# waldstein94/Stratified-Transformer

Measured on AMD Instinct MI355X. Metric: points/sec through StratifiedAttention fwd+bwd, 100k-pt scene, higher is better.
Workload: dtype f32

## Files before the change

stratified_transformer_amd/csrc/cell_attn.hip:

```cpp
#include "cell_common.h"

namespace p2 {


template <typename T>
__device__ __forceinline__ void stage_table_t(T *lds, const T *__restrict__ tab, int L, int h, int head) {
    const int total = 3 * L * 16;
    for (int x = threadIdx.x; x < total; x += blockDim.x) {
        const int i = x % 16, r = (x / 16) % L, ax = x / (16 * L);
        lds[x] = tab[(((size_t)r * h + head) * 16 + i) * 3 + ax];
    }
}
template <int TS, typename T>
__device__ __forceinline__ void stage_tables(T *lds, const T *__restrict__ table_q, const T *__restrict__ table_k, const T *__restrict__ table_v, int L,
                                             int h, int head) {
    stage_table_t<T>(lds, table_q, L, h, head);
    stage_table_t<T>(lds + TS, table_k, L, h, head);
    stage_table_t<T>(lds + 2 * TS, table_v, L, h, head);
    __syncthreads();
}

template <int LCAP>
struct TabGeo {
    static constexpr int TS = 3 * LCAP * 16;
    static constexpr size_t bytes(size_t elem) { return (size_t)3 * TS * elem; }
};
struct RowOff {
    int o0, o1, o2;
};
__device__ __forceinline__ RowOff row_off(unsigned w, int L, int c) {
    RowOff r;
    r.o0 = (int)(w & 255u) * 16 + 4 * c;
    r.o1 = (int)(L + ((w >> 8) & 255u)) * 16 + 4 * c;
    r.o2 = (int)(2 * L + ((w >> 16) & 255u)) * 16 + 4 * c;
    return r;
}
template <int OFF>
__device__ __forceinline__ float4 tsum_at(const float *lds, RowOff r) {
    return add4(add4(*reinterpret_cast<const float4 *>(lds + OFF + r.o0), *reinterpret_cast<const float4 *>(lds + OFF + r.o1)),
                *reinterpret_cast<const float4 *>(lds + OFF + r.o2));
}

struct Rows3 {
    float4 a, b, c;
};
template <int OFF, typename T>
__device__ __forceinline__ Rows3 rows_at(const T *lds, RowOff r) {
    Rows3 x;
    x.a = ld_row4(lds + OFF + r.o0);
    x.b = ld_row4(lds + OFF + r.o1);
    x.c = ld_row4(lds + OFF + r.o2);
    return x;
}
typedef float f32x2c __attribute__((ext_vector_type(2)));
__device__ __forceinline__ float4 padd4(float4 a, float4 b) {
    const f32x2c lo = f32x2c{a.x, a.y} + f32x2c{b.x, b.y}, hi = f32x2c{a.z, a.w} + f32x2c{b.z, b.w};
    return make_float4(lo.x, lo.y, hi.x, hi.y);
}
__device__ __forceinline__ float4 pfma4(float s, float4 a, float4 acc) {
    const f32x2c ss = f32x2c{s, s};
    const f32x2c lo = __builtin_elementwise_fma(ss, f32x2c{a.x, a.y}, f32x2c{acc.x, acc.y});
    const f32x2c hi = __builtin_elementwise_fma(ss, f32x2c{a.z, a.w}, f32x2c{acc.z, acc.w});
    return make_float4(lo.x, lo.y, hi.x, hi.y);
}
__device__ __forceinline__ float4 rsum(Rows3 r) { return padd4(padd4(r.a, r.b), r.c); }
__device__ __forceinline__ f32x2c pdot_acc(float4 a, float4 b, f32x2c acc) {
    acc = __builtin_elementwise_fma(f32x2c{a.x, a.y}, f32x2c{b.x, b.y}, acc);
    return __builtin_elementwise_fma(f32x2c{a.z, a.w}, f32x2c{b.z, b.w}, acc);
}
__device__ __forceinline__ float pdot4(float4 a, float4 b) {
    const f32x2c r = pdot_acc(a, b, f32x2c{0.f, 0.f});
    return r.x + r.y;
}

template <int NPMAX, typename F>
__device__ __forceinline__ void dispatch_passes(int np, F f) {
    if (np <= 2) f(std::integral_constant<int, 2>{});
    else if (np == 3) f(std::integral_constant<int, 3>{});
    else if (np == 4 || NPMAX <= 4) f(std::integral_constant<int, 4>{});
    else if constexpr (NPMAX > 4) {
        if (np <= 6) f(std::integral_constant<int, 6>{});
        else f(std::integral_constant<int, 8>{});
    }
}

template <typename TT, bool PK>
struct LaneCtx {
    const TT *lds;
    int L, lane, p, c, head, h, C, hoff, rs_packed;
    float qscale;
    __device__ __forceinline__ int rs() const { return PK ? rs_packed : C; }
    template <typename RT>
    __device__ __forceinline__ float4 q_row4(const RT *q, int i) const {
        if constexpr (PK) return scaled_row4<RT>(q + (size_t)i * rs_packed + hoff, qscale);
        else return ld_row4(q + (size_t)i * C + hoff);
    }
};
template <typename TT, bool PK>
__device__ __forceinline__ LaneCtx<TT, PK> make_lane_ctx(const TT *lds, int h, int L, int rs, float qscale) {
    LaneCtx<TT, PK> x;
    x.lds = lds;
    x.L = L;
    x.h = h;
    x.head = blockIdx.y;
    x.C = h * 16;
    x.rs_packed = rs;
    x.qscale = qscale;
    x.lane = threadIdx.x & 63;
    x.p = x.lane >> 2;
    x.c = x.lane & 3;
    x.hoff = x.head * 16 + 4 * x.c;
    return x;
}

template <int NPA, typename RT, typename T, bool PK>
__device__ __forceinline__ void load_key_rows(const LaneCtx<T, PK> &x, const CellBufs &cb, const RT *__restrict__ rows, int j0, int nvalid,
                                              float4 (&r4)[NPA]) {
    unsigned keys[NPA];
    bload_words<NPA>(cb.key, (j0 + x.p * NPA) * 4, keys);
#pragma unroll
    for (int t = 0; t < NPA; t++) {
        const float4 r = ld_row4(rows + (size_t)keys[t] * x.rs() + x.hoff);
        r4[t] = t < nvalid ? r : make_float4(0.f, 0.f, 0.f, 0.f);
    }
}

template <int NPA, int TS, typename RT, typename T, bool PK>
__device__ __forceinline__ void fwd_sweep_logits(const LaneCtx<T, PK> &x, const CellTask &ct, const CellBufs &cb, rsrc_t rs_p,
                                                 const RT *__restrict__ q, const RT *__restrict__ k, float *__restrict__ ml,
                                                 int ch, bool single, int j0, int nkc) {
    const int p = x.p, c = x.c;
    const int nvalid = min(max(nkc - p * NPA, 0), NPA);
    float4 k4[NPA];
    load_key_rows<NPA, RT, T, PK>(x, cb, k, j0, nvalid, k4);
    int ids = (int)bload_u32(cb.qid, x.lane * 4);
    int i_nx = __builtin_amdgcn_readlane(ids, 0);
    float4 q4_nx = x.q_row4(q, i_nx);
    unsigned w_nx[NPA];
    bload_words<NPA>(cb.rel, (j0 + p * NPA) * 4, w_nx);
    for (int il = 0; il < ct.nq; il++) {
        const int i = i_nx;
        const float4 q4 = q4_nx;
        unsigned w[NPA];
#pragma unroll
        for (int t = 0; t < NPA; t++) w[t] = w_nx[t];
        const int roff = (il * ct.nk + j0 + p * NPA) * 4;
        if (((il + 1) & 63) == 0) ids = (int)bload_u32(cb.qid, (il + 1 + x.lane) * 4);
        i_nx = __builtin_amdgcn_readlane(ids, (il + 1) & 63);
        q4_nx = x.q_row4(q, i_nx);
        bload_words<NPA>(cb.rel, roff + ct.nk * 4, w_nx);
        float lg[NPA];
        float mx = -INFINITY;
        RowOff ro = row_off(w[0], x.L, c);
        Rows3 rq = rows_at<0, T>(x.lds, ro), rk = rows_at<TS, T>(x.lds, ro);
#pragma unroll
        for (int t = 0; t < NPA; t++) {
            Rows3 rq1 = rq, rk1 = rk;
            if (t + 1 < NPA) {
                ro = row_off(w[t + 1], x.L, c);
                rq1 = rows_at<0, T>(x.lds, ro);
                rk1 = rows_at<TS, T>(x.lds, ro);
            }
            const f32x2c d2 = pdot_acc(k4[t], rsum(rk), pdot_acc(q4, rsum(rq), pdot_acc(q4, k4[t], f32x2c{0.f, 0.f})));
            const float s = quad_sum(d2.x + d2.y);
            lg[t] = (t < nvalid && !(w[t] >> 31)) ? s : -INFINITY;
            mx = fmaxf(mx, lg[t]);
            rq = rq1;
            rk = rk1;
            __builtin_amdgcn_sched_barrier(0);
        }
        mx = slots_max16(mx);
        if (single) {
            float sum = 0.f;
#pragma unroll
            for (int t = 0; t < NPA; t++) {
                lg[t] = __expf(lg[t] - mx);
                sum += lg[t];
            }
            const float inv = 1.0f / slots_sum16(sum);
#pragma unroll
            for (int t = 0; t < NPA; t++) lg[t] *= inv;
            if (c == 0) bstore_floats<NPA>(rs_p, roff, lg, nvalid);
        } else {
            float *st = ml + ((size_t)i * x.h + x.head) * 2;
            const float m_old = ch ? st[0] : -INFINITY, l_old = ch ? st[1] : 0.f;
            const float m_new = fmaxf(m_old, mx);
            float sum = 0.f;
#pragma unroll
            for (int t = 0; t < NPA; t++) sum += __expf(lg[t] - m_new);
            if (c == 0) bstore_floats<NPA>(rs_p, roff, lg, nvalid);
            sum = slots_sum16(sum);
            if (x.lane == 0) {
                st[0] = m_new;
                st[1] = (m_old == -INFINITY ? 0.f : l_old * __expf(m_old - m_new)) + sum;
            }
        }
    }
}

template <int NPA, int TS, typename RT, typename T, bool PK>
__device__ __forceinline__ void fwd_sweep_values(const LaneCtx<T, PK> &x, const CellTask &ct, const CellBufs &cb, rsrc_t rs_p,
                                                 const RT *__restrict__ v, const float *__restrict__ ml, float *__restrict__ out,
                                                 int ch, bool single, int j0, int nkc) {
    const int p = x.p, c = x.c;
    const int nvalid = min(max(nkc - p * NPA, 0), NPA);
    float4 v4[NPA];
    load_key_rows<NPA, RT, T, PK>(x, cb, v, j0, nvalid, v4);
    unsigned w_nx[NPA];
    float a_nx[NPA];
    bload_words<NPA>(cb.rel, (j0 + p * NPA) * 4, w_nx);
    bload_floats<NPA>(rs_p, (j0 + p * NPA) * 4, a_nx);
    int ids = (int)bload_u32(cb.qid, x.lane * 4);
    for (int il = 0; il < ct.nq; il++) {
        if (il && (il & 63) == 0) ids = (int)bload_u32(cb.qid, (il + x.lane) * 4);
        const int i = __builtin_amdgcn_readlane(ids, il & 63);
        const int roff = (il * ct.nk + j0 + p * NPA) * 4;
        unsigned w[NPA];
        float a[NPA];
#pragma unroll
        for (int t = 0; t < NPA; t++) {
            w[t] = w_nx[t];
            a[t] = a_nx[t];
        }
        bload_words<NPA>(cb.rel, roff + ct.nk * 4, w_nx);
        bload_floats<NPA>(rs_p, roff + ct.nk * 4, a_nx);
        if (!single) {
            const float *st = ml + ((size_t)i * x.h + x.head) * 2;
            const float m = st[0], inv = 1.0f / st[1];
#pragma unroll
            for (int t = 0; t < NPA; t++) a[t] = __expf(a[t] - m) * inv;
            if (c == 0) bstore_floats<NPA>(rs_p, roff, a, nvalid);
        }
        float4 acc = make_float4(0.f, 0.f, 0.f, 0.f);
        Rows3 rv = rows_at<2 * TS, T>(x.lds, row_off(w[0], x.L, c));
#pragma unroll
        for (int t = 0; t < NPA; t++) {
            Rows3 rv1 = rv;
            if (t + 1 < NPA) rv1 = rows_at<2 * TS, T>(x.lds, row_off(w[t + 1], x.L, c));
            const float at = t < nvalid ? a[t] : 0.f;
            acc = pfma4(at, padd4(rsum(rv), v4[t]), acc);
            rv = rv1;
            __builtin_amdgcn_sched_barrier(0);
        }
        const float4 tot = slots_sum16_4(acc);
        if (p == 0) {
            float *o = out + (size_t)i * x.C + x.hoff;
            stg4(o, ch ? add4(tot, ldg4(o)) : tot);
        }
    }
}

template <int NP, int LCAP, typename RT, typename T, bool PK>
__global__ __launch_bounds__(CA_WAVES * 64) void cell_fwd_kernel(pointops2_cell_plan pl, int h, int L, const RT *__restrict__ q,
                                                                 const RT *__restrict__ k, const RT *__restrict__ v, int rs, float qscale,
                                                                 const T *__restrict__ table_q, const T *__restrict__ table_k,
                                                                 const T *__restrict__ table_v, float *__restrict__ out,
                                                                 float *__restrict__ ml, float *__restrict__ pbuf, size_t plane) {
    constexpr int TS = TabGeo<LCAP>::TS;
    extern __shared__ float lds_raw[];
    T *lds = reinterpret_cast<T *>(lds_raw);
    const LaneCtx<T, PK> x = make_lane_ctx<T, PK>(lds, h, L, rs, qscale);
    const int wave = __builtin_amdgcn_readfirstlane(threadIdx.x >> 6);
    stage_tables<TS, T>(lds, table_q, table_k, table_v, L, h, x.head);
    const int nC = share_count(pl, pl.counts[0]);
    float *pb = pbuf + (size_t)x.head * plane;
    const int slots = gridDim.x * CA_WAVES, slot = blockIdx.x * CA_WAVES + wave;
    for (int round = 0; round * slots < nC; round++) {
        const int task = snake_task(round, slot, slots);
        if (task >= nC) continue;
        const CellTask ct = cell_task(pl, share_task(pl, task));
        const int nch = (ct.nk + 16 * NP - 1) / (16 * NP);
        const CellBufs cb = make_cell_bufs(pl, ct);
        const rsrc_t rs_p = tile_rsrc(pb, ct);
        for (int ch = 0; ch < nch; ch++) {
            const int j0 = ch * 16 * NP, nkc = min(16 * NP, ct.nk - j0);
            dispatch_passes<NP>((nkc + 15) >> 4, [&](auto tag) {
                fwd_sweep_logits<decltype(tag)::value, TS, RT, T, PK>(x, ct, cb, rs_p, q, k, ml, ch, nch == 1, j0, nkc);
            });
        }
        for (int ch = 0; ch < nch; ch++) {
            const int j0 = ch * 16 * NP, nkc = min(16 * NP, ct.nk - j0);
            dispatch_passes<NP>((nkc + 15) >> 4, [&](auto tag) {
                fwd_sweep_values<decltype(tag)::value, TS, RT, T, PK>(x, ct, cb, rs_p, v, ml, out, ch, nch == 1, j0, nkc);
            });
        }
    }
}

template <int NPA, typename T, bool PK>
__device__ __forceinline__ void flush_key_pass(float *scr, float4 acc, rsrc_t rs_key, int j0, int t, int nkc, float *__restrict__ grad,
                                               const LaneCtx<T, PK> &x) {
    *reinterpret_cast<float4 *>(scr + x.p * 16 + 4 * x.c) = acc;
    __builtin_amdgcn_s_waitcnt(0xC07F);
    __builtin_amdgcn_wave_barrier();
#pragma unroll
    for (int kk = 0; kk < 4; kk++) {
        const int s = (x.lane >> 4) + 4 * kk;
        const int jl = s * NPA + t;
        const int key = (int)bload_u32(rs_key, (j0 + jl) * 4);
        if (jl < nkc) unsafeAtomicAdd(grad + (size_t)key * x.rs() + x.head * 16 + (x.lane & 15), scr[s * 16 + (x.lane & 15)]);
    }
    __builtin_amdgcn_s_waitcnt(0xC07F);
    __builtin_amdgcn_wave_barrier();
}

template <int NPA, int TS, typename RT, typename T, bool PK>
__device__ __forceinline__ void bwd_sweep_values(const LaneCtx<T, PK> &x, const CellTask &ct, const CellBufs &cb, rsrc_t rs_p, rsrc_t rs_g,
                                                 float *scr, const float *__restrict__ go, const float *__restrict__ out,
                                                 const RT *__restrict__ v, float *__restrict__ grad_v, int j0, int nkc) {
    const int p = x.p, c = x.c;
    const int nvalid = min(max(nkc - p * NPA, 0), NPA);
    float4 v4[NPA], dv4[NPA];
    load_key_rows<NPA, RT, T, PK>(x, cb, v, j0, nvalid, v4);
#pragma unroll
    for (int t = 0; t < NPA; t++) dv4[t] = make_float4(0.f, 0.f, 0.f, 0.f);
    unsigned w_nx[NPA];
    float a_nx[NPA];
    bload_words<NPA>(cb.rel, (j0 + p * NPA) * 4, w_nx);
    bload_floats<NPA>(rs_p, (j0 + p * NPA) * 4, a_nx);
    int ids = (int)bload_u32(cb.qid, x.lane * 4);
    int i_nx = __builtin_amdgcn_readlane(ids, 0);
    float4 go_nx = ldg4(go + (size_t)i_nx * x.C + x.hoff), o_nx = ldg4(out + (size_t)i_nx * x.C + x.hoff);
    for (int il = 0; il < ct.nq; il++) {
        const int roff = (il * ct.nk + j0 + p * NPA) * 4;
        const float4 go4 = go_nx, o4 = o_nx;
        unsigned w[NPA];
        float a[NPA];
#pragma unroll
        for (int t = 0; t < NPA; t++) {
            w[t] = w_nx[t];
            a[t] = t < nvalid ? a_nx[t] : 0.f;
        }
        if (((il + 1) & 63) == 0) ids = (int)bload_u32(cb.qid, (il + 1 + x.lane) * 4);
        i_nx = __builtin_amdgcn_readlane(ids, (il + 1) & 63);
        go_nx = ldg4(go + (size_t)i_nx * x.C + x.hoff);
        o_nx = ldg4(out + (size_t)i_nx * x.C + x.hoff);
        bload_words<NPA>(cb.rel, roff + ct.nk * 4, w_nx);
        bload_floats<NPA>(rs_p, roff + ct.nk * 4, a_nx);
        const float delta = quad_sum(pdot4(go4, o4));
        float gs[NPA];
        Rows3 rv = rows_at<2 * TS, T>(x.lds, row_off(w[0], x.L, c));
#pragma unroll
        for (int t = 0; t < NPA; t++) {
            Rows3 rv1 = rv;
            if (t + 1 < NPA) rv1 = rows_at<2 * TS, T>(x.lds, row_off(w[t + 1], x.L, c));
            const float ga = quad_sum(pdot4(go4, padd4(rsum(rv), v4[t])));
            gs[t] = a[t] * (ga - delta);
            dv4[t] = pfma4(a[t], go4, dv4[t]);
            rv = rv1;
            __builtin_amdgcn_sched_barrier(0);
        }
        if (c == 0) bstore_floats<NPA>(rs_g, roff, gs, nvalid);
    }
#pragma unroll
    for (int t = 0; t < NPA; t++) flush_key_pass<NPA, T, PK>(scr, dv4[t], cb.key, j0, t, nkc, grad_v, x);
}

template <int NPA, int TS, typename RT, typename T, bool PK>
__device__ __forceinline__ void bwd_sweep_keys(const LaneCtx<T, PK> &x, const CellTask &ct, const CellBufs &cb, rsrc_t rs_g, float *scr,
                                               const RT *__restrict__ q, const RT *__restrict__ k, float *__restrict__ grad_q,
                                               float *__restrict__ grad_k, int ch, int j0, int nkc) {
    const int p = x.p, c = x.c;
    const int nvalid = min(max(nkc - p * NPA, 0), NPA);
    float4 k4[NPA], dk4[NPA];
    load_key_rows<NPA, RT, T, PK>(x, cb, k, j0, nvalid, k4);
#pragma unroll
    for (int t = 0; t < NPA; t++) dk4[t] = make_float4(0.f, 0.f, 0.f, 0.f);
    unsigned w_nx[NPA];
    float g_nx[NPA];
    bload_words<NPA>(cb.rel, (j0 + p * NPA) * 4, w_nx);
    bload_floats<NPA>(rs_g, (j0 + p * NPA) * 4, g_nx);
    int ids = (int)bload_u32(cb.qid, x.lane * 4);
    int i_nx = __builtin_amdgcn_readlane(ids, 0);
    float4 q_nx = x.q_row4(q, i_nx);
    for (int il = 0; il < ct.nq; il++) {
        const int i = i_nx;
        const int roff = (il * ct.nk + j0 + p * NPA) * 4;
        const float4 q4 = q_nx;
        unsigned w[NPA];
        float g[NPA];
#pragma unroll
        for (int t = 0; t < NPA; t++) {
            w[t] = w_nx[t];
            g[t] = t < nvalid ? g_nx[t] : 0.f;
        }
        if (((il + 1) & 63) == 0) ids = (int)bload_u32(cb.qid, (il + 1 + x.lane) * 4);
        i_nx = __builtin_amdgcn_readlane(ids, (il + 1) & 63);
        q_nx = x.q_row4(q, i_nx);
        bload_words<NPA>(cb.rel, roff + ct.nk * 4, w_nx);
        bload_floats<NPA>(rs_g, roff + ct.nk * 4, g_nx);
        float4 dq = make_float4(0.f, 0.f, 0.f, 0.f);
        RowOff ro = row_off(w[0], x.L, c);
        Rows3 rq = rows_at<0, T>(x.lds, ro), rk = rows_at<TS, T>(x.lds, ro);
#pragma unroll
        for (int t = 0; t < NPA; t++) {
            Rows3 rq1 = rq, rk1 = rk;
            if (t + 1 < NPA) {
                ro = row_off(w[t + 1], x.L, c);
                rq1 = rows_at<0, T>(x.lds, ro);
                rk1 = rows_at<TS, T>(x.lds, ro);
            }
            dq = pfma4(g[t], padd4(rsum(rq), k4[t]), dq);
            dk4[t] = pfma4(g[t], padd4(rsum(rk), q4), dk4[t]);
            rq = rq1;
            rk = rk1;
            __builtin_amdgcn_sched_barrier(0);
        }
        float4 tot = slots_sum16_4(dq);
        if constexpr (PK) tot = make_float4(tot.x * x.qscale, tot.y * x.qscale, tot.z * x.qscale, tot.w * x.qscale);
        if (p == 0) {
            float *o = grad_q + (size_t)i * x.rs() + x.hoff;
            stg4(o, ch ? add4(tot, ldg4(o)) : tot);
        }
    }
#pragma unroll
    for (int t = 0; t < NPA; t++) flush_key_pass<NPA, T, PK>(scr, dk4[t], cb.key, j0, t, nkc, grad_k, x);
}

template <int NP, int LCAP, typename RT, typename T, bool PK>
__global__ __launch_bounds__(CA_WAVES_BWD * 64) void cell_bwd_kernel(pointops2_cell_plan pl, int h, int L, const float *__restrict__ go,
                                                                 const RT *__restrict__ q, const RT *__restrict__ k,
                                                                 const RT *__restrict__ v, int rs, float qscale, const float *__restrict__ out,
                                                                 const T *__restrict__ table_q, const T *__restrict__ table_k,
                                                                 const T *__restrict__ table_v, const float *__restrict__ pbuf,
                                                                 float *__restrict__ gsbuf, size_t plane, float *__restrict__ grad_q,
                                                                 float *__restrict__ grad_k, float *__restrict__ grad_v) {
    constexpr int TS = TabGeo<LCAP>::TS;
    extern __shared__ float lds_raw[];
    T *lds = reinterpret_cast<T *>(lds_raw);
    const LaneCtx<T, PK> x = make_lane_ctx<T, PK>(lds, h, L, rs, qscale);
    const int wave = __builtin_amdgcn_readfirstlane(threadIdx.x >> 6);
    float *scr = reinterpret_cast<float *>(lds + 3 * TS) + wave * 256;
    stage_tables<TS, T>(lds, table_q, table_k, table_v, L, h, x.head);
    const int nC = share_count(pl, pl.counts[0]);
    const float *pb = pbuf + (size_t)x.head * plane;
    float *gb = gsbuf + (size_t)x.head * plane;
    const int slots = gridDim.x * CA_WAVES_BWD, slot = blockIdx.x * CA_WAVES_BWD + wave;
    for (int round = 0; round * slots < nC; round++) {
        const int task = snake_task(round, slot, slots);
        if (task >= nC) continue;
        const CellTask ct = cell_task(pl, share_task(pl, task));
        const int nch = (ct.nk + 16 * NP - 1) / (16 * NP);
        const CellBufs cb = make_cell_bufs(pl, ct);
        const rsrc_t rs_p = tile_rsrc(pb, ct), rs_g = tile_rsrc(gb, ct);
        for (int ch = 0; ch < nch; ch++) {
            const int j0 = ch * 16 * NP, nkc = min(16 * NP, ct.nk - j0);
            dispatch_passes<NP>((nkc + 15) >> 4, [&](auto tag) {
                bwd_sweep_values<decltype(tag)::value, TS, RT, T, PK>(x, ct, cb, rs_p, rs_g, scr, go, out, v, grad_v, j0, nkc);
            });
        }
        for (int ch = 0; ch < nch; ch++) {
            const int j0 = ch * 16 * NP, nkc = min(16 * NP, ct.nk - j0);
            dispatch_passes<NP>((nkc + 15) >> 4, [&](auto tag) {
                bwd_sweep_keys<decltype(tag)::value, TS, RT, T, PK>(x, ct, cb, rs_g, scr, q, k, grad_q, grad_k, ch, j0, nkc);
            });
        }
    }
}

struct CFixScale {
    float mul, inv;
};
__device__ __forceinline__ CFixScale c_row_scale(unsigned maxbits, int n) {
    CFixScale sc;
    if (maxbits >= 0x7f800000u) {
        sc.mul = 0.f;
        sc.inv = __uint_as_float(0x7fc00000u);
        return sc;
    }
    const int E = (int)(maxbits >> 23) - 126;
    const int bits_n = 32 - __clz(max(n, 1));
    const int S = max(-126, min(126, 30 - bits_n - E));
    sc.mul = __uint_as_float((unsigned)(S + 127) << 23);
    sc.inv = __uint_as_float((unsigned)(127 - S) << 23);
    return sc;
}

constexpr int CT_WAVES = 8;

template <int TA>
struct CellTableGeo {
    static constexpr int LP = TA * 16;
    static constexpr int ROW = 3 * LP + 16;
    static constexpr size_t walk_bytes() { return (size_t)CT_WAVES * 4 * ROW * 4; }
    static constexpr size_t sum_bytes() { return (size_t)LP * 48 * 4; }
    static constexpr size_t lds_bytes() { return walk_bytes() > sum_bytes() ? walk_bytes() : sum_bytes(); }
};

template <int TA, bool BYKEY, bool SC, typename XT>
__device__ __forceinline__ void cell_table_grad_body(const pointops2_cell_plan &pl, int h, int L, const float *__restrict__ wbuf, size_t plane,
                                                     const XT *__restrict__ X, int xs, float xscale, float *__restrict__ grad_table) {
    constexpr int D = 16;
    constexpr int MAXP = BYKEY ? 4 : 8;
    using G = CellTableGeo<TA>;
    extern __shared__ float lds[];
    const int wave = __builtin_amdgcn_readfirstlane(threadIdx.x >> 6), lane = threadIdx.x & 63;
    const int head = blockIdx.y;
    const int p = lane >> 2, c = lane & 3;
    const int kq = lane >> 4, col = lane & 15;
    int *hist = reinterpret_cast<int *>(lds) + wave * 4 * G::ROW;
    const float *wb = wbuf + (size_t)head * plane;

    f32x4c acc[TA][3];
#pragma unroll
    for (int bt = 0; bt < TA; bt++)
#pragma unroll
        for (int ax = 0; ax < 3; ax++) acc[bt][ax] = f32x4c{0.f, 0.f, 0.f, 0.f};
    for (int x = lane; x < 4 * G::ROW; x += 64) hist[x] = 0;

    const int nC = BYKEY ? pl.counts[4] : share_count(pl, pl.counts[0]);
    const int slots = gridDim.x * CT_WAVES, slot = blockIdx.x * CT_WAVES + wave;
    for (int round = 0; round * slots < nC; round++) {
        const int task = snake_task(round, slot, slots);
        if (task >= nC) continue;
        CellTask ct;
        if (BYKEY) {
            const int c0 = __builtin_amdgcn_readfirstlane(pl.parent_first[task]), c1 = __builtin_amdgcn_readfirstlane(pl.parent_first[task + 1]);
            ct.qs = __builtin_amdgcn_readfirstlane(pl.cell_qstart[c0]);
            ct.nq = __builtin_amdgcn_readfirstlane(pl.cell_qstart[c1]) - ct.qs;
            ct.kb = __builtin_amdgcn_readfirstlane(pl.cell_kbase[c0]);
            ct.nk = __builtin_amdgcn_readfirstlane(pl.cell_kbase[c0 + 1]) - ct.kb;
            ct.pbase = __builtin_amdgcn_readfirstlane(pl.cell_pbase[c0]);
        } else {
            ct = cell_task(pl, share_task(pl, task));
        }
        const CellBufs cb = make_cell_bufs(pl, ct);
        const rsrc_t rs_rel = cb.rel, rs_w = tile_rsrc(wb, ct), rs_row = BYKEY ? cb.key : cb.qid;
        const int nrows = BYKEY ? ct.nk : ct.nq, nent = BYKEY ? ct.nq : ct.nk;
        auto entry_off = [&](int r0, int ent) -> int { return (BYKEY ? ent * ct.nk + r0 + c : (r0 + c) * ct.nk + ent) * 4; };
        auto consume = [&](int r0, int e0, float xv, unsigned (&wr)[MAXP], float (&wt)[MAXP]) {
            const int ne = min(nent - e0, 16 * MAXP);
            const bool row_ok = r0 + c < nrows;
            unsigned mxb = 0u;
#pragma unroll
            for (int t = 0; t < MAXP; t++) {
                const bool live = row_ok && e0 + 16 * t + p < nent && !(wr[t] >> 31);
                wt[t] = live ? wt[t] : 0.f;
                mxb = max(mxb, __float_as_uint(fabsf(wt[t])));
            }
            const CFixScale sc = c_row_scale(wave_max_u32(mxb), ne);
            int *myh = hist + c * G::ROW;
#pragma unroll
            for (int t = 0; t < MAXP; t++) {
                if (16 * t < ne && wt[t] != 0.f) {
                    const int v = __float2int_rn(wt[t] * sc.mul);
                    atomicAdd(&myh[wr[t] & 255u], v);
                    atomicAdd(&myh[G::LP + ((wr[t] >> 8) & 255u)], v);
                    atomicAdd(&myh[2 * G::LP + ((wr[t] >> 16) & 255u)], v);
                }
            }
            __builtin_amdgcn_s_waitcnt(0xC07F);
            __builtin_amdgcn_wave_barrier();
            const float b = xv * sc.inv;
#pragma unroll
            for (int bt = 0; bt < TA; bt++)
#pragma unroll
                for (int ax = 0; ax < 3; ax++) {
                    const float a = (float)__hip_atomic_exchange(&hist[kq * G::ROW + ax * G::LP + bt * 16 + col], 0, __ATOMIC_RELAXED,
                                                                 __HIP_MEMORY_SCOPE_WORKGROUP);
                    acc[bt][ax] = __builtin_amdgcn_mfma_f32_16x16x4f32(a, b, acc[bt][ax], 0, 0, 0);
                }
            __builtin_amdgcn_s_waitcnt(0xC07F);
            __builtin_amdgcn_wave_barrier();
        };
        unsigned wr_n[MAXP];
        float wt_n[MAXP];
#pragma unroll
        for (int t = 0; t < MAXP; t++) {
            wr_n[t] = 0x80000000u;
            wt_n[t] = 0.f;
            if (16 * t < nent) {
                wr_n[t] = bload_u32(rs_rel, entry_off(0, 16 * t + p));
                wt_n[t] = bload_f32(rs_w, entry_off(0, 16 * t + p));
            }
        }
        int pt_n = (int)bload_u32(rs_row, kq * 4);
        float xv_n = SC ? scaled_elem<XT>(X + (size_t)pt_n * xs + head * D + col, xscale) : ld_elem(X + (size_t)pt_n * xs + head * D + col);
        pt_n = (int)bload_u32(rs_row, (4 + kq) * 4);
        for (int r0 = 0; r0 < nrows; r0 += 4) {
            unsigned wr[MAXP];
            float wt[MAXP];
#pragma unroll
            for (int t = 0; t < MAXP; t++) {
                wr[t] = wr_n[t];
                wt[t] = wt_n[t];
            }
            const float xv = r0 + kq < nrows ? xv_n : 0.f;
            xv_n = SC ? scaled_elem<XT>(X + (size_t)pt_n * xs + head * D + col, xscale) : ld_elem(X + (size_t)pt_n * xs + head * D + col);
            pt_n = (int)bload_u32(rs_row, (r0 + 8 + kq) * 4);
#pragma unroll
            for (int t = 0; t < MAXP; t++)
                if (16 * t < nent) {
                    wr_n[t] = bload_u32(rs_rel, entry_off(r0 + 4, 16 * t + p));
                    wt_n[t] = bload_f32(rs_w, entry_off(r0 + 4, 16 * t + p));
                }
            consume(r0, 0, xv, wr, wt);
            for (int e0 = 16 * MAXP; e0 < nent; e0 += 16 * MAXP) {
#pragma unroll
                for (int t = 0; t < MAXP; t++) {
                    wr[t] = bload_u32(rs_rel, entry_off(r0, e0 + 16 * t + p));
                    wt[t] = bload_f32(rs_w, entry_off(r0, e0 + 16 * t + p));
                }
                consume(r0, e0, xv, wr, wt);
            }
        }
    }
    __syncthreads();
    float *sum = lds;
    for (int w = 0; w < CT_WAVES; w++) {
        if (wave == w) {
#pragma unroll
            for (int bt = 0; bt < TA; bt++)
#pragma unroll
                for (int ax = 0; ax < 3; ax++)
#pragma unroll
                    for (int reg = 0; reg < 4; reg++) {
                        float *d = &sum[((bt * 16 + kq * 4 + reg) * 16 + col) * 3 + ax];
                        *d = w ? *d + acc[bt][ax][reg] : acc[bt][ax][reg];
                    }
        }
        __syncthreads();
    }
    for (int x = threadIdx.x; x < L * 48; x += CT_WAVES * 64) {
        const float val = sum[x];
        if (val != 0.f) unsafeAtomicAdd(grad_table + ((size_t)(x / 48) * h + head) * 48 + x % 48, val);
    }
}

template <int TA, typename T, bool PK>
__global__ __launch_bounds__(CT_WAVES * 64) void cell_table_grad3_kernel(pointops2_cell_plan pl, int h, int L, const float *__restrict__ gsbuf,
                                                                         const float *__restrict__ pbuf, size_t plane,
                                                                         const T *__restrict__ q, const T *__restrict__ k,
                                                                         const float *__restrict__ grad_out, float *__restrict__ gtq,
                                                                         float *__restrict__ gtk, float *__restrict__ gtv, int rs, float qscale) {
    const int xs = PK ? rs : h * 16;
    if (blockIdx.z == 0) cell_table_grad_body<TA, true, false, T>(pl, h, L, gsbuf, plane, k, xs, 1.0f, gtk);
    else if (blockIdx.z == 1) cell_table_grad_body<TA, false, PK, T>(pl, h, L, gsbuf, plane, q, xs, qscale, gtq);
    else cell_table_grad_body<TA, false, false, float>(pl, h, L, pbuf, plane, grad_out, h * 16, 1.0f, gtv);
}

static const char *cell_refusal(const pointops2_cell_plan *plan, int hdim, int L, bool backward) {
    if (hdim != 16) return "cell_attention: d != 16";
    if (backward && (L < 1 || L > 80)) return "cell_attention backward: table rows L must be in 1..80";
    if (L < 1) return "cell_attention: no table rows";
    if (L != plan->table_rows)
        return backward ? "cell_attention backward: the tables' row count differs from the plan's table_rows"
                        : "cell_attention: the tables' row count differs from the plan's table_rows";
    if (L > 160) return "cell_attention: more than 160 table rows (use the operators)";
    return nullptr;
}

static int cell_fwd_variant(const pointops2_cell_plan *plan, int h, int hdim, int L, bool bf16, const char **why) {
    *why = nullptr;
    if (plan == nullptr || plan->n_points <= 0) return POINTOPS2_CELL_FWD_NONE;
    if ((*why = cell_refusal(plan, hdim, L, false)) != nullptr) return POINTOPS2_CELL_FWD_ERROR;
    if (L > 80) return POINTOPS2_CELL_FWD_VALU160;
    if (!bf16) {
        const double avg_queries = (double)plan->n_pairs / (double)(plan->n_keyslots > 0 ? plan->n_keyslots : 1);
        if (!((long long)plan->n_points * h >= 96000 && avg_queries < 15.0)) return L <= 64 ? POINTOPS2_CELL_FWD_MFMA64 : POINTOPS2_CELL_FWD_MFMA80;
    }
    return POINTOPS2_CELL_FWD_VALU80;
}

template <int LCAP, typename RT, typename TT, bool PK>
static void launch_valu_fwd(hipStream_t st, const pointops2_cell_plan *plan, int h, int L, const CellRows<RT> &r, const CellTables<TT> &t, float *out, float *ml,
                            float *pbuf) {
    const size_t lds = TabGeo<LCAP>::bytes(sizeof(TT));
    allow_big_lds(cell_fwd_kernel<CA_NP, LCAP, RT, TT, PK>, lds);
    const dim3 grid(cell_grid_x(1, plan->n_cells, h, CA_WAVES), h);
    hipLaunchKernelGGL((cell_fwd_kernel<CA_NP, LCAP, RT, TT, PK>), grid, dim3(CA_WAVES * 64), lds, st, *plan, h, L, r.q, r.k, r.v, r.rs, r.scale, t.q, t.k, t.v, out,
                       ml, pbuf, (size_t)plan->n_pairs);
}

template <typename RT, typename TT, bool PK>
static void launch_cell_fwd(hipStream_t st, const pointops2_cell_plan *plan, int h, int hdim, int L, const CellRows<RT> &r, const CellTables<TT> &t, float *out,
                            float *ml, float *pbuf) {
    const char *why;
    const int variant = cell_fwd_variant(plan, h, hdim, L, !std::is_same<TT, float>::value, &why);
    if (why != nullptr) { set_error(why); return; }
    if (variant == POINTOPS2_CELL_FWD_NONE) return;
    if constexpr (std::is_same<TT, float>::value) {
        if (variant == POINTOPS2_CELL_FWD_MFMA64 || variant == POINTOPS2_CELL_FWD_MFMA80) {
            cell_fwd_mfma_launch(st, variant, plan, h, L, RowTag<RT>::code, PK, CellRows<void>{r.q, r.k, r.v, r.rs, r.scale}, t, out, pbuf);
            check_launch();
            return;
        }
    }
    if (variant == POINTOPS2_CELL_FWD_VALU80) launch_valu_fwd<80, RT, TT, PK>(st, plan, h, L, r, t, out, ml, pbuf);
    else launch_valu_fwd<160, RT, TT, PK>(st, plan, h, L, r, t, out, ml, pbuf);
    check_launch();
}

template <typename RT, typename TT, bool PK>
static void launch_cell_bwd(hipStream_t st, const pointops2_cell_plan *plan, int h, int hdim, int L, const float *grad_out, const CellRows<RT> &r, const float *out,
                            const CellTables<TT> &t, const float *pbuf, float *gsbuf, const CellGrads &g, const CellGrads &gt) {
    if (plan == nullptr || plan->n_points <= 0) return;
    if (const char *why = cell_refusal(plan, hdim, L, true)) { set_error(why); return; }
    const size_t lds = TabGeo<80>::bytes(sizeof(TT)) + (size_t)CA_WAVES_BWD * 256 * sizeof(float);
    allow_big_lds(cell_bwd_kernel<CA_NP_BWD, 80, RT, TT, PK>, lds);
    const size_t plane = (size_t)plan->n_pairs;
    hipLaunchKernelGGL((cell_bwd_kernel<CA_NP_BWD, 80, RT, TT, PK>), dim3(cell_grid_x(1, plan->n_cells, h, CA_WAVES_BWD), h),
                       dim3(CA_WAVES_BWD * 64), lds, st, *plan, h, L, grad_out, r.q, r.k, r.v, r.rs, r.scale, out, t.q, t.k, t.v, pbuf, gsbuf, plane, g.q, g.k, g.v);
    const dim3 grid3(cell_grid_x(1, plan->n_cells, h, CT_WAVES), h, 3), tblock(CT_WAVES * 64);
    if (L <= 64) hipLaunchKernelGGL((cell_table_grad3_kernel<4, RT, PK>), grid3, tblock, CellTableGeo<4>::lds_bytes(), st, *plan, h, L, gsbuf, pbuf, plane, r.q, r.k,
                                    grad_out, gt.q, gt.k, gt.v, r.rs, r.scale);
    else hipLaunchKernelGGL((cell_table_grad3_kernel<5, RT, PK>), grid3, tblock, CellTableGeo<5>::lds_bytes(), st, *plan, h, L, gsbuf, pbuf, plane, r.q, r.k, grad_out,
                            gt.q, gt.k, gt.v, r.rs, r.scale);
    check_launch();
}

template <typename RT>
static CellRows<RT> packed_rows(const void *qkv, int h, float scale) {
    const RT *r = static_cast<const RT *>(qkv);
    return {r, r + h * 16, r + 2 * h * 16, 3 * h * 16, scale};
}

}

using namespace p2;

extern "C" {

int pointops2_cell_forward_variant(const pointops2_cell_plan *plan, int h, int hdim, int L, int bf16) {
    const char *why;
    return cell_fwd_variant(plan, h, hdim, L, bf16 != 0, &why);
}

void cell_attention_forward_launcher(const pointops2_cell_plan *plan, int h, int hdim, int L, const float *q, const float *k,
                                     const float *v, const float *table_q, const float *table_k, const float *table_v, float *out,
                                     float *ml, float *pbuf) {
    launch_cell_fwd<float, float, false>(begin_launch().stream, plan, h, hdim, L, {q, k, v, h * 16, 1.0f}, {table_q, table_k, table_v}, out, ml, pbuf);
}
void cell_attention_backward_launcher(const pointops2_cell_plan *plan, int h, int hdim, int L, const float *grad_out, const float *q,
                                      const float *k, const float *v, const float *out, const float *table_q, const float *table_k,
                                      const float *table_v, const float *pbuf, float *gsbuf, float *grad_q, float *grad_k,
                                      float *grad_v, float *grad_table_q, float *grad_table_k, float *grad_table_v) {
    launch_cell_bwd<float, float, false>(begin_launch().stream, plan, h, hdim, L, grad_out, {q, k, v, h * 16, 1.0f}, out, {table_q, table_k, table_v}, pbuf, gsbuf,
                                         {grad_q, grad_k, grad_v}, {grad_table_q, grad_table_k, grad_table_v});
}
void cell_attention_forward_bf16_launcher(const pointops2_cell_plan *plan, int h, int hdim, int L, const uint16_t *q, const uint16_t *k,
                                          const uint16_t *v, const uint16_t *table_q, const uint16_t *table_k, const uint16_t *table_v,
                                          float *out, float *ml, float *pbuf) {
    launch_cell_fwd<bf16_t, bf16_t, false>(begin_launch().stream, plan, h, hdim, L, {q, k, v, h * 16, 1.0f}, {table_q, table_k, table_v}, out, ml, pbuf);
}
void cell_attention_backward_bf16_launcher(const pointops2_cell_plan *plan, int h, int hdim, int L, const float *grad_out, const uint16_t *q,
                                           const uint16_t *k, const uint16_t *v, const float *out, const uint16_t *table_q,
                                           const uint16_t *table_k, const uint16_t *table_v, const float *pbuf, float *gsbuf, float *grad_q,
                                           float *grad_k, float *grad_v, float *grad_table_q, float *grad_table_k, float *grad_table_v) {
    launch_cell_bwd<bf16_t, bf16_t, false>(begin_launch().stream, plan, h, hdim, L, grad_out, {q, k, v, h * 16, 1.0f}, out, {table_q, table_k, table_v}, pbuf, gsbuf,
                                           {grad_q, grad_k, grad_v}, {grad_table_q, grad_table_k, grad_table_v});
}

void cell_attention_qkv_forward_launcher(const pointops2_cell_plan *plan, int h, int hdim, int L, const void *qkv, int row_type, float scale,
                                         const float *table_q, const float *table_k, const float *table_v, float *out, float *ml, float *pbuf) {
    const hipStream_t st = begin_launch().stream;
    if (!with_row_type(row_type, [&](auto tag) {
        using RT = typename decltype(tag)::type;
        launch_cell_fwd<RT, float, true>(st, plan, h, hdim, L, packed_rows<RT>(qkv, h, scale), {table_q, table_k, table_v}, out, ml, pbuf);
    })) set_error("cell_attention_qkv: unknown row_type");
}
void cell_attention_qkv_backward_launcher(const pointops2_cell_plan *plan, int h, int hdim, int L, const float *grad_out, const void *qkv, int row_type,
                                          float scale, const float *out, const float *table_q, const float *table_k, const float *table_v,
                                          const float *pbuf, float *gsbuf, float *grad_qkv, float *grad_table_q, float *grad_table_k,
                                          float *grad_table_v) {
    const hipStream_t st = begin_launch().stream;
    if (!with_row_type(row_type, [&](auto tag) {
        using RT = typename decltype(tag)::type;
        launch_cell_bwd<RT, float, true>(st, plan, h, hdim, L, grad_out, packed_rows<RT>(qkv, h, scale), out, {table_q, table_k, table_v}, pbuf, gsbuf,
                                         {grad_qkv, grad_qkv + h * 16, grad_qkv + 2 * h * 16}, {grad_table_q, grad_table_k, grad_table_v});
    })) set_error("cell_attention_qkv backward: unknown row_type");
}

}
```

Baseline: 8.887 million.

## Defer per-query stores one iteration and batch key loads in gradient flush

Stores of softmax probabilities, output rows, gradient scores and dQ rows now happen one iteration later, so each store overlaps the next query's compute instead of trailing it. An explicit vmcnt wait at the top of each loop, with the loops pinned to unroll 1, makes the prefetch and store timing predictable. The key-gradient flush now loads all key indices once up front and then does the scatter atomics, instead of reloading them for every slot. The cost is extra live registers for the previous iteration's values, and the full vmem wait may serialize loads that could otherwise have stayed in flight.

```diff
diff --git a/stratified_transformer_amd/csrc/cell_attn.hip b/stratified_transformer_amd/csrc/cell_attn.hip
--- a/stratified_transformer_amd/csrc/cell_attn.hip
+++ b/stratified_transformer_amd/csrc/cell_attn.hip
@@ -113,6 +113,16 @@
     return x;
 }
 
+__device__ __forceinline__ void wait_vmem() {
+    asm volatile("" ::: "memory");
+    __builtin_amdgcn_s_waitcnt(0x0F70);
+}
+__device__ __forceinline__ int next_query_ids(rsrc_t qid, int off) {
+    const int ids = (int)bload_u32(qid, off);
+    wait_vmem();
+    return ids;
+}
+
 template <int NPA, typename RT, typename T, bool PK>
 __device__ __forceinline__ void load_key_rows(const LaneCtx<T, PK> &x, const CellBufs &cb, const RT *__restrict__ rows, int j0, int nvalid,
                                               float4 (&r4)[NPA]) {
@@ -138,17 +148,23 @@
     float4 q4_nx = x.q_row4(q, i_nx);
     unsigned w_nx[NPA];
     bload_words<NPA>(cb.rel, (j0 + p * NPA) * 4, w_nx);
+    float lg_pv[NPA];
+#pragma unroll
+    for (int t = 0; t < NPA; t++) lg_pv[t] = 0.f;
+#pragma unroll 1
     for (int il = 0; il < ct.nq; il++) {
+        wait_vmem();
         const int i = i_nx;
         const float4 q4 = q4_nx;
         unsigned w[NPA];
 #pragma unroll
         for (int t = 0; t < NPA; t++) w[t] = w_nx[t];
         const int roff = (il * ct.nk + j0 + p * NPA) * 4;
-        if (((il + 1) & 63) == 0) ids = (int)bload_u32(cb.qid, (il + 1 + x.lane) * 4);
+        if (((il + 1) & 63) == 0) ids = next_query_ids(cb.qid, (il + 1 + x.lane) * 4);
         i_nx = __builtin_amdgcn_readlane(ids, (il + 1) & 63);
         q4_nx = x.q_row4(q, i_nx);
         bload_words<NPA>(cb.rel, roff + ct.nk * 4, w_nx);
+        if (single && il && c == 0) bstore_floats<NPA>(rs_p, roff - ct.nk * 4, lg_pv, nvalid);
         float lg[NPA];
         float mx = -INFINITY;
         RowOff ro = row_off(w[0], x.L, c);
@@ -179,8 +195,7 @@
             }
             const float inv = 1.0f / slots_sum16(sum);
 #pragma unroll
-            for (int t = 0; t < NPA; t++) lg[t] *= inv;
-            if (c == 0) bstore_floats<NPA>(rs_p, roff, lg, nvalid);
+            for (int t = 0; t < NPA; t++) lg_pv[t] = lg[t] * inv;
         } else {
             float *st = ml + ((size_t)i * x.h + x.head) * 2;
             const float m_old = ch ? st[0] : -INFINITY, l_old = ch ? st[1] : 0.f;
@@ -196,6 +211,7 @@
             }
         }
     }
+    if (single && ct.nq > 0 && c == 0) bstore_floats<NPA>(rs_p, ((ct.nq - 1) * ct.nk + j0 + p * NPA) * 4, lg_pv, nvalid);
 }
 
 template <int NPA, int TS, typename RT, typename T, bool PK>
@@ -211,8 +227,16 @@
     bload_words<NPA>(cb.rel, (j0 + p * NPA) * 4, w_nx);
     bload_floats<NPA>(rs_p, (j0 + p * NPA) * 4, a_nx);
     int ids = (int)bload_u32(cb.qid, x.lane * 4);
+    float4 tot_pv = make_float4(0.f, 0.f, 0.f, 0.f);
+    int i_pv = 0;
+    auto store_out = [&](int i, float4 tot) {
+        float *o = out + (size_t)i * x.C + x.hoff;
+        stg4(o, ch ? add4(tot, ldg4(o)) : tot);
+    };
+#pragma unroll 1
     for (int il = 0; il < ct.nq; il++) {
-        if (il && (il & 63) == 0) ids = (int)bload_u32(cb.qid, (il + x.lane) * 4);
+        wait_vmem();
+        if (il && (il & 63) == 0) ids = next_query_ids(cb.qid, (il + x.lane) * 4);
         const int i = __builtin_amdgcn_readlane(ids, il & 63);
         const int roff = (il * ct.nk + j0 + p * NPA) * 4;
         unsigned w[NPA];
@@ -224,6 +248,7 @@
         }
         bload_words<NPA>(cb.rel, roff + ct.nk * 4, w_nx);
         bload_floats<NPA>(rs_p, roff + ct.nk * 4, a_nx);
+        if (il && p == 0) store_out(i_pv, tot_pv);
         if (!single) {
             const float *st = ml + ((size_t)i * x.h + x.head) * 2;
             const float m = st[0], inv = 1.0f / st[1];
@@ -242,12 +267,10 @@
             rv = rv1;
             __builtin_amdgcn_sched_barrier(0);
         }
-        const float4 tot = slots_sum16_4(acc);
-        if (p == 0) {
-            float *o = out + (size_t)i * x.C + x.hoff;
-            stg4(o, ch ? add4(tot, ldg4(o)) : tot);
-        }
-    }
+        tot_pv = slots_sum16_4(acc);
+        i_pv = i;
+    }
+    if (ct.nq > 0 && p == 0) store_out(i_pv, tot_pv);
 }
 
 template <int NP, int LCAP, typename RT, typename T, bool PK>
@@ -288,20 +311,25 @@
 }
 
 template <int NPA, typename T, bool PK>
-__device__ __forceinline__ void flush_key_pass(float *scr, float4 acc, rsrc_t rs_key, int j0, int t, int nkc, float *__restrict__ grad,
-                                               const LaneCtx<T, PK> &x) {
-    *reinterpret_cast<float4 *>(scr + x.p * 16 + 4 * x.c) = acc;
-    __builtin_amdgcn_s_waitcnt(0xC07F);
-    __builtin_amdgcn_wave_barrier();
-#pragma unroll
-    for (int kk = 0; kk < 4; kk++) {
-        const int s = (x.lane >> 4) + 4 * kk;
-        const int jl = s * NPA + t;
-        const int key = (int)bload_u32(rs_key, (j0 + jl) * 4);
-        if (jl < nkc) unsafeAtomicAdd(grad + (size_t)key * x.rs() + x.head * 16 + (x.lane & 15), scr[s * 16 + (x.lane & 15)]);
-    }
-    __builtin_amdgcn_s_waitcnt(0xC07F);
-    __builtin_amdgcn_wave_barrier();
+__device__ __forceinline__ void flush_key_grads(float *scr, const float4 (&acc)[NPA], rsrc_t rs_key, int j0, int nkc, float *__restrict__ grad,
+                                                const LaneCtx<T, PK> &x) {
+    unsigned keys[4][NPA];
+#pragma unroll
+    for (int kk = 0; kk < 4; kk++) bload_words<NPA>(rs_key, (j0 + ((x.lane >> 4) + 4 * kk) * NPA) * 4, keys[kk]);
+    wait_vmem();
+#pragma unroll
+    for (int t = 0; t < NPA; t++) {
+        *reinterpret_cast<float4 *>(scr + x.p * 16 + 4 * x.c) = acc[t];
+        __builtin_amdgcn_s_waitcnt(0xC07F);
+        __builtin_amdgcn_wave_barrier();
+#pragma unroll
+        for (int kk = 0; kk < 4; kk++) {
+            const int s = (x.lane >> 4) + 4 * kk;
+            if (s * NPA + t < nkc) unsafeAtomicAdd(grad + (size_t)keys[kk][t] * x.rs() + x.head * 16 + (x.lane & 15), scr[s * 16 + (x.lane & 15)]);
+        }
+        __builtin_amdgcn_s_waitcnt(0xC07F);
+        __builtin_amdgcn_wave_barrier();
+    }
 }
 
 template <int NPA, int TS, typename RT, typename T, bool PK>
@@ -321,7 +349,12 @@
     int ids = (int)bload_u32(cb.qid, x.lane * 4);
     int i_nx = __builtin_amdgcn_readlane(ids, 0);
     float4 go_nx = ldg4(go + (size_t)i_nx * x.C + x.hoff), o_nx = ldg4(out + (size_t)i_nx * x.C + x.hoff);
+    float gs_pv[NPA];
+#pragma unroll
+    for (int t = 0; t < NPA; t++) gs_pv[t] = 0.f;
+#pragma unroll 1
     for (int il = 0; il < ct.nq; il++) {
+        wait_vmem();
         const int roff = (il * ct.nk + j0 + p * NPA) * 4;
         const float4 go4 = go_nx, o4 = o_nx;
         unsigned w[NPA];
@@ -331,29 +364,28 @@
             w[t] = w_nx[t];
             a[t] = t < nvalid ? a_nx[t] : 0.f;
         }
-        if (((il + 1) & 63) == 0) ids = (int)bload_u32(cb.qid, (il + 1 + x.lane) * 4);
+        if (((il + 1) & 63) == 0) ids = next_query_ids(cb.qid, (il + 1 + x.lane) * 4);
         i_nx = __builtin_amdgcn_readlane(ids, (il + 1) & 63);
         go_nx = ldg4(go + (size_t)i_nx * x.C + x.hoff);
         o_nx = ldg4(out + (size_t)i_nx * x.C + x.hoff);
         bload_words<NPA>(cb.rel, roff + ct.nk * 4, w_nx);
         bload_floats<NPA>(rs_p, roff + ct.nk * 4, a_nx);
+        if (il && c == 0) bstore_floats<NPA>(rs_g, roff - ct.nk * 4, gs_pv, nvalid);
         const float delta = quad_sum(pdot4(go4, o4));
-        float gs[NPA];
         Rows3 rv = rows_at<2 * TS, T>(x.lds, row_off(w[0], x.L, c));
 #pragma unroll
         for (int t = 0; t < NPA; t++) {
             Rows3 rv1 = rv;
             if (t + 1 < NPA) rv1 = rows_at<2 * TS, T>(x.lds, row_off(w[t + 1], x.L, c));
             const float ga = quad_sum(pdot4(go4, padd4(rsum(rv), v4[t])));
-            gs[t] = a[t] * (ga - delta);
+            gs_pv[t] = a[t] * (ga - delta);
             dv4[t] = pfma4(a[t], go4, dv4[t]);
             rv = rv1;
             __builtin_amdgcn_sched_barrier(0);
         }
-        if (c == 0) bstore_floats<NPA>(rs_g, roff, gs, nvalid);
-    }
-#pragma unroll
-    for (int t = 0; t < NPA; t++) flush_key_pass<NPA, T, PK>(scr, dv4[t], cb.key, j0, t, nkc, grad_v, x);
+    }
+    if (ct.nq > 0 && c == 0) bstore_floats<NPA>(rs_g, ((ct.nq - 1) * ct.nk + j0 + p * NPA) * 4, gs_pv, nvalid);
+    flush_key_grads<NPA, T, PK>(scr, dv4, cb.key, j0, nkc, grad_v, x);
 }
 
 template <int NPA, int TS, typename RT, typename T, bool PK>
@@ -373,7 +405,15 @@
     int ids = (int)bload_u32(cb.qid, x.lane * 4);
     int i_nx = __builtin_amdgcn_readlane(ids, 0);
     float4 q_nx = x.q_row4(q, i_nx);
+    float4 tot_pv = make_float4(0.f, 0.f, 0.f, 0.f);
+    int i_pv = 0;
+    auto store_dq = [&](int i, float4 tot) {
+        float *o = grad_q + (size_t)i * x.rs() + x.hoff;
+        stg4(o, ch ? add4(tot, ldg4(o)) : tot);
+    };
+#pragma unroll 1
     for (int il = 0; il < ct.nq; il++) {
+        wait_vmem();
         const int i = i_nx;
         const int roff = (il * ct.nk + j0 + p * NPA) * 4;
         const float4 q4 = q_nx;
@@ -384,11 +424,12 @@
             w[t] = w_nx[t];
             g[t] = t < nvalid ? g_nx[t] : 0.f;
         }
-        if (((il + 1) & 63) == 0) ids = (int)bload_u32(cb.qid, (il + 1 + x.lane) * 4);
+        if (((il + 1) & 63) == 0) ids = next_query_ids(cb.qid, (il + 1 + x.lane) * 4);
         i_nx = __builtin_amdgcn_readlane(ids, (il + 1) & 63);
         q_nx = x.q_row4(q, i_nx);
         bload_words<NPA>(cb.rel, roff + ct.nk * 4, w_nx);
         bload_floats<NPA>(rs_g, roff + ct.nk * 4, g_nx);
+        if (il && p == 0) store_dq(i_pv, tot_pv);
         float4 dq = make_float4(0.f, 0.f, 0.f, 0.f);
         RowOff ro = row_off(w[0], x.L, c);
         Rows3 rq = rows_at<0, T>(x.lds, ro), rk = rows_at<TS, T>(x.lds, ro);
@@ -408,13 +449,11 @@
         }
         float4 tot = slots_sum16_4(dq);
         if constexpr (PK) tot = make_float4(tot.x * x.qscale, tot.y * x.qscale, tot.z * x.qscale, tot.w * x.qscale);
-        if (p == 0) {
-            float *o = grad_q + (size_t)i * x.rs() + x.hoff;
-            stg4(o, ch ? add4(tot, ldg4(o)) : tot);
-        }
-    }
-#pragma unroll
-    for (int t = 0; t < NPA; t++) flush_key_pass<NPA, T, PK>(scr, dk4[t], cb.key, j0, t, nkc, grad_k, x);
+        tot_pv = tot;
+        i_pv = i;
+    }
+    if (ct.nq > 0 && p == 0) store_dq(i_pv, tot_pv);
+    flush_key_grads<NPA, T, PK>(scr, dk4, cb.key, j0, nkc, grad_k, x);
 }
 
 template <int NP, int LCAP, typename RT, typename T, bool PK>
```

Result: faster. 9.087 million, median of 6 (+2.3%).
